# pyranha-labs/hypergrep

Measured on AMD Instinct MI355X. Metric: GiB/s scanned (256 patterns, 32 GiB synthetic log per GPU, text resident in HBM), higher is better.
Workload: dtype u8

## Files before the change

### hypergrep_amd/build.py

```python
from __future__ import annotations

import os
import shutil
import subprocess
import sys

PKG = os.path.dirname(os.path.abspath(__file__))
REPO = os.path.dirname(PKG)
CSRC = os.path.join(PKG, "csrc")
LIB_DIR = os.path.join(PKG, "lib")
LIB = os.path.join(LIB_DIR, "libhyperscanner.so")
LIBHS_NAME = "libhs.so.5"
OBJ = os.path.join(REPO, "build", "obj")
EXTRA = os.environ.get("HG_BUILD_DEFINES", "").split()
if os.environ.get("HG_BUILD_OUT"):
    LIB = os.path.abspath(os.environ["HG_BUILD_OUT"])
    LIB_DIR = os.path.dirname(LIB)
    OBJ = LIB + ".obj"
    LIBHS_NAME = os.path.basename(LIB) + ".libhs.so.5"

HIP_SOURCES = ["hg_stream.hip", "hg_kernels.hip", "hg_always_on.hip", "hg_huge.hip", "hg_som.hip", "hg_comb.hip", "hg_flows.hip", "hg_batch.hip", "hg_engine.hip", "hg_capi.hip", "hg_shim.hip", "hg_hsface.hip"]
CXX_SOURCES = ["hg_compile.cpp"]
HEADERS = ["hg_mem.h", "hg_db.h", "hg_core.h", "hg_post.h", "hg_engine.h", "hg_compile.h", "hg_synth.h", "hg_confirm_dev.h", "hg_sink_dev.h", "hg_tables_dev.h", "hg_som.h", "hg_comb.h", "hg_flows.h", "hg_flow_rules.h", "hg_batch.h", "hg_batch_launch.h"]

# ... 44 lines not shown

def _merge_resources() -> None:
    import json

    table = {}
    for src in KERNEL_SOURCES:
        path = os.path.join(OBJ, src + ".resources.json")
        if os.path.exists(path):
            with open(path, encoding="utf-8") as f:
                table.update(json.load(f))
    with open(os.path.join(LIB_DIR, "kernel_resources.json"), "w", encoding="utf-8") as f:
        json.dump(table, f, indent=1, sort_keys=True)
    for kernel, res in table.items():
        if kernel.startswith("_Z16hg_stream_kernelILi") and "ELb0ELi0E" in kernel and res.get("ScratchSize [bytes/lane]", 0) > 16:
            raise RuntimeError(f"{kernel} uses {res['ScratchSize [bytes/lane]']} bytes of scratch per lane: the streaming hot path must stay in registers")
        if "hg_som_kernel" in kernel and res.get("ScratchSize [bytes/lane]", 0) > 0:
            raise RuntimeError(f"{kernel} uses {res['ScratchSize [bytes/lane]']} bytes of scratch per lane: the start-of-match walks keep their state in registers / LDS")
        if "hg_minlen_kernel" in kernel and res.get("ScratchSize [bytes/lane]", 0) > 0:
            raise RuntimeError(f"{kernel} uses {res['ScratchSize [bytes/lane]']} bytes of scratch per lane: the match-length walks keep their state in registers / LDS")
        if "hg_flow_som_kernel" in kernel and res.get("ScratchSize [bytes/lane]", 0) > 0:
            raise RuntimeError(f"{kernel} uses {res['ScratchSize [bytes/lane]']} bytes of scratch per lane: the stream-mode start-of-match lanes keep their starts in device memory")
        if "hg_block_batch_kernel" in kernel and (res.get("ScratchSize [bytes/lane]", 0) > 0 or res.get("VGPRs Spill", 0) > 0):
            raise RuntimeError(f"{kernel} uses {res['ScratchSize [bytes/lane]']} bytes of scratch per lane, {res['VGPRs Spill']} spilled VGPRs: the batched block scan keeps its automaton state in registers")
        if "hg_comb_kernel" in kernel and res.get("ScratchSize [bytes/lane]", 0) > 0:
            raise RuntimeError(f"{kernel} uses {res['ScratchSize [bytes/lane]']} bytes of scratch per lane: the combination pass keeps its evaluation stack in a register")


def build(verbose: bool = False, force: bool = False) -> str:
    from concurrent.futures import ThreadPoolExecutor

    os.makedirs(OBJ, exist_ok=True)
    os.makedirs(LIB_DIR, exist_ok=True)
    hipcc = _hipcc()
    common_deps = [os.path.join(CSRC, h) for h in HEADERS] + [os.path.join(REPO, "include", "hypergrep_amd.h")]
    objs, jobs = [], []
    for src in HIP_SOURCES + CXX_SOURCES:
        path = os.path.join(CSRC, src)
        if not os.path.exists(path):
            continue
        obj = os.path.join(OBJ, src + ".o")
        objs.append(obj)
        if force or _stale(obj, [path] + common_deps):
            if src.endswith(".hip"):
                cmd = [hipcc, "--offload-arch=gfx950", "-O3", "-std=c++17", "-fPIC", "-Wall", "-Wno-pass-failed"] + EXTRA + ["-c", path, "-o", obj]
            else:
                cmd = ["g++", "-O2", "-std=c++17", "-fPIC", "-Wall", "-Wextra", "-c", path, "-o", obj]
# ... 34 lines not shown
```

### hypergrep_amd/csrc/hg_engine.h

```cpp
#pragma once
#include <hip/hip_runtime.h>

#include <memory>
#include <string>

#include "../../include/hypergrep_amd.h"
#include "hg_compile.h"
#include "hg_core.h"
#include "hg_post.h"

#ifndef HG_STREAM_WG_WAVES
#define HG_STREAM_WG_WAVES 8
#endif
constexpr uint32_t HG_STREAM_WG_WAVES_DEFAULT = HG_STREAM_WG_WAVES;

constexpr uint32_t HG_CONFIRM_SPLIT = 4;
constexpr uint32_t HG_DEFER_SHARDS = 64;

struct HgDeferred {
  uint64_t pos;
  uint32_t pattern;
  uint32_t rank;
};
enum { HG_ST_MINLEN_KEPT = 16, HG_ST_FIN_TOTAL = 24, HG_ST_SELECTED = 28, HG_ST_FINAL = 32, HG_ST_WORDS = 36, HG_ST_ZERO_WORDS = 32,
       HG_ST_BLOCK_DONE = 40 };
enum { HG_CNT_CANDS = 0, HG_CNT_HITS = 1, HG_CNT_CAND_NEED = 2, HG_CNT_HIT_NEED = 3, HG_CNT_DEFER_NEED = 4,
       HG_CNT_HITS_WRAPPED = 5,
       HG_CNT_JOIN_TILES = 6,
       HG_CNT_WORDS = 8,
       HG_CNT_CURSOR0 = 64,
       HG_CNT_CURSORS = 64,
       HG_ST_ALLOC_WORDS = 128 };
constexpr uint32_t HG_STREAM_GRAB = 2 * HG_STREAM_WG_WAVES_DEFAULT;

constexpr uint32_t HG_FIN_MAX_BUCKETS = 1u << 22;
constexpr uint32_t HG_FIN_BUCKET_CAP = 4096;
constexpr uint32_t HG_FIN_MEDIUM_CAP = 512;

#ifndef HG_CONFIRM_THREADS
#define HG_CONFIRM_THREADS 128
#endif



struct HgStreamArgs {
  const uint8_t *text;
  uint64_t nbytes, tile_begin, tile_end;
  HgDbView db;
  const uint32_t *filter;
  const HgSlotInfo *ext;
  HgTileSum *sums;
  HgCand *cands;
  uint32_t *seg_count;
  uint32_t cand_seg_cap, filter_log2;
  uint32_t weights_a, weights_b;
  uint32_t filter_wide;
  uint32_t dense;
  uint32_t weights_c;
  uint32_t alone;
  uint32_t cursor_slot;
  uint32_t *counters;
};

struct HgConfirmArgs {
  const uint8_t *text;
  uint64_t nbytes, tile_begin, tile_end, bs1;
// ... 204 lines not shown
```

### hypergrep_amd/csrc/hg_engine.hip

```cpp
#include <algorithm>
#include <array>
#include <cstdio>
#include <cstdlib>
#include <cstring>
#include <memory>

#include "hg_engine.h"
#include "hg_mem.h"

#include <rocprim/rocprim.hpp>

bool hg_launch_stream(const HgStreamArgs &a, uint32_t grid, hipStream_t stream);
bool hg_launch_stream_join(const HgStreamArgs &a, uint32_t grid, hipStream_t stream);
int hg_stream_blocks_per_cu(uint32_t filter_log2, uint32_t filter_wide, uint32_t dense);
__global__ void hg_tile_reduce_kernel(const HgTileSum *sums, uint64_t tile_begin, uint64_t tile_end, uint64_t bs1, HgTileElem *agg);
__global__ void hg_tile_spine_kernel(const HgTileElem *agg, uint32_t nblocks, uint64_t bs1, HgTileBase *block_base, HgTileBase *state);
__global__ void hg_tile_apply_kernel(const HgTileSum *sums, uint64_t tile_begin, uint64_t tile_end, uint64_t bs1, const HgTileBase *block_base,
                                     HgTileBase *bases);
__global__ void hg_tile_inner_kernel(const uint8_t *text, HgTileSum *sums, uint64_t tile_begin, uint64_t tile_end, uint64_t bs1);
__global__ void hg_verify_kernel(HgConfirmArgs a);
__global__ void hg_confirm_fast_kernel(HgConfirmArgs a, uint32_t blocks_per_mode);
__global__ void hg_confirm_generic_kernel(HgConfirmArgs a);
__global__ void hg_always_on_kernel(HgConfirmArgs a, uint32_t first, uint32_t last);
__global__ void hg_always_on_fast_kernel(HgConfirmArgs a);
__global__ void hg_always_on_finish_kernel(HgConfirmArgs a);
__global__ void hg_block_mark_kernel(HgConfirmArgs a, uint32_t *pattern_flags);
__global__ void hg_block_scan_kernel(HgConfirmArgs a, const uint32_t *pattern_flags);
__global__ void hg_block_small_kernel(HgDbView db, const uint8_t *h_text, uint32_t length, HgHit *h_out, uint32_t seg_cap, uint32_t *h_counts, uint32_t *d_done,
                                      uint32_t *h_flag, uint32_t seq, uint32_t ppw);
__global__ void hg_reset_kernel(uint32_t *state, uint32_t state_words, HgTileBase *final_state, uint64_t carry_start, uint64_t first_piece, uint32_t *fill, uint32_t nb, uint32_t *defer_count,
                                uint32_t ndefer);
__global__ void hg_fin_sort_small_kernel(const HgHit *hits, uint32_t *idx, const uint32_t *fill, uint32_t b_lo, uint32_t b_hi, uint32_t cap, uint32_t id_bits,
                                         uint32_t to_bits, uint32_t *kept_count, uint32_t *big_list, uint32_t *big_count, uint32_t big_stride);
template <uint32_t LCAP, bool IN_LDS>
__global__ void hg_fin_sort_big_kernel(const HgHit *hits, uint32_t *idx, const uint32_t *fill, const uint32_t *big_list, const uint32_t *big_count, uint32_t cap,
                                       uint32_t id_bits, uint32_t to_bits, uint32_t *kept_count, uint32_t *overflow, uint64_t *scratch_key, uint32_t *scratch_idx);
template <uint32_t THREADS>
__global__ void hg_fin_scan_kernel(uint32_t *kept_count, uint32_t b_lo, uint32_t b_hi, uint32_t *total, const uint32_t *fill, uint32_t cap, uint32_t *part, uint32_t epoch);
__global__ void hg_confirm_literal_kernel(HgConfirmArgs a);
__global__ void hg_verify_lean_kernel(HgConfirmArgs a);
__global__ void hg_fin_gather_kernel(const HgHit *hits, const HgHitAux *aux, const uint32_t *idx, const uint32_t *kept_base, const uint32_t *total, uint32_t b_lo,
                                     uint32_t b_hi, uint32_t cap, HgHit *oh, HgHitAux *oa);
__global__ void hg_key_kernel(const HgHit *hits, const HgHitAux *aux, const HgPattern *patterns, uint32_t n, uint64_t *key, uint32_t *idx);
__global__ void hg_line_key_kernel(const HgHit *hits, const uint32_t *perm, uint32_t n, uint64_t *key);
__global__ void hg_offset_kernel(uint32_t *idx, uint32_t n, uint32_t add);
__global__ void hg_key_packed_kernel(const HgHit *hits, const HgHitAux *aux, const HgPattern *patterns, uint32_t n, uint32_t id_bits, uint32_t to_bits,
                                     uint64_t *key, uint32_t *idx);
__global__ void hg_keep_kernel(const HgHit *hits, const HgHitAux *aux, const uint32_t *perm, const HgPattern *patterns, uint32_t n, uint8_t *keep);
__global__ void hg_scatter_kernel(const HgHit *hits, const HgHitAux *aux, const uint32_t *perm, const uint8_t *keep, const uint32_t *pos, uint32_t n,
                                  HgHit *oh, HgHitAux *oa, uint32_t *count);

size_t hg_huge_lds_bytes(uint32_t nw_max, uint32_t stage_cap);
bool hg_launch_confirm_huge(const HgConfirmArgs &a, uint32_t grid, uint32_t nw_max, uint32_t stage_cap, void *claim, uint32_t claim_mask, hipStream_t stream);
bool hg_launch_always_on_huge(const HgConfirmArgs &a, uint32_t grid, uint32_t nw_max, uint32_t stage_cap, uint32_t first, uint32_t last, hipStream_t stream);
bool hg_launch_block_huge(const HgConfirmArgs &a, uint32_t grid, uint32_t nw_max, uint32_t stage_cap, const uint32_t *pattern_flags, hipStream_t stream);

namespace {
constexpr int TS_BLOCK_TILES = 1024;
constexpr int STREAM_WG_WAVES = HG_STREAM_WG_WAVES;

template <typename T>
hipError_t upload(void **dst, const std::vector<T> &src, const char *name) {
  size_t bytes = std::max<size_t>(src.size() * sizeof(T), 16);
// ... 198 lines not shown
  (void)rocprim::exclusive_scan(nullptr, t2, d_keep_, d_perm_a_, 0u, n, rocprim::plus<uint32_t>(), hipStream_t(nullptr));
  size_t t3 = 0;
  (void)rocprim::merge(nullptr, t3, d_key_a_, d_key_a_, d_key_b_, d_perm_a_, d_perm_a_, d_perm_b_, n, n, rocprim::less<uint64_t>(), hipStream_t(nullptr));
  size_t need = std::max(std::max(t1, t2), t3) + 256;
  if (need > temp_bytes_) {
    hgmem::dev_free(d_temp_, "d_temp_");
    d_temp_ = nullptr;
    HG_TRY(hgmem::dev_alloc(&d_temp_, need, "d_temp_"), "workspace alloc (sort)");
    temp_bytes_ = need;
  }
  return HG_OK;
}

int HgScanner::ensure(uint64_t nbytes) {
  uint64_t ntiles = std::max<uint64_t>((nbytes + HG_TILE_BYTES - 1) / HG_TILE_BYTES, 1);
  auto re = [&](auto *&ptr, size_t count, const char *name) { return fail(realloc_dev(ptr, count, name), "workspace alloc"); };
  if (ntiles > cap_tiles_) {
    uint64_t nblocks = (ntiles + TS_BLOCK_TILES - 1) / TS_BLOCK_TILES;
    if (re(d_sums_, ntiles, "d_sums_") || re(d_bases_, ntiles + 1, "d_bases_") || re(d_agg_, nblocks, "d_agg_") || re(d_block_base_, nblocks, "d_block_base_")) return HG_ERR_HIP;
    cap_tiles_ = ntiles;
  }
  if (!d_seg_count_) {
    max_segs_ = static_cast<uint32_t>(num_cus_) * 16;
    if (re(d_seg_count_, max_segs_, "d_seg_count_") || re(d_seg_count2_, max_segs_, "d_seg_count2_") || re(d_defer_count_, HG_CONFIRM_MODES * HG_DEFER_SHARDS, "d_defer_count_")) return HG_ERR_HIP;
  }
  uint64_t want = std::max<uint64_t>(nbytes / 1024, 1u << 16);
  if (cand_cap_ < want && alloc_cands(want)) return HG_ERR_HIP;
  if (hit_cap_ < want && alloc_hits(want)) return HG_ERR_HIP;
  return HG_OK;
}

enum { HG_SPLIT = 1000, HG_GROWN = 1001 };

struct HgScanner::PassPlan {
  const uint8_t *text;
  uint64_t nbytes, bs1, ntiles;
  PassRange range;
  bool block_mode, has_anchored;
  hipStream_t stream, side;
  uint32_t id_bits, to_bits, fin_shift = 10, fin_nb = 1, fin_cap;
  bool bucketed;
  uint32_t nchunks = 1;
  bool piped, split;
  uint64_t chunk_tiles;
  std::array<uint64_t, kMaxChunks + 1> cut;
  uint32_t wgs_alone, wgs_shared, joiner_wgs, wgs = 1;
  uint32_t cand_seg_cap[2];
// ... 221 lines not shown
  if (p.block_mode) {
    HG_TRY(hipMemsetAsync(d_pflags_, 0, db_->patterns.size() * 4, side), "memset pattern flags");
    if (p.has_anchored) hipLaunchKernelGGL(hg_block_mark_kernel, dim3(segs_c), dim3(256), 0, side, ca, d_pflags_);
    always_blocks = std::max<uint32_t>(static_cast<uint32_t>((db_->patterns.size() + 255) / 256), std::min<uint32_t>(db_->nhuge, 1024u));
    ca.hit_seg_cap = hit_cap_ / always_blocks;
    hipLaunchKernelGGL(hg_block_scan_kernel, dim3(static_cast<uint32_t>((db_->patterns.size() + 255) / 256)), dim3(256), 0, side, ca, d_pflags_);
    if (db_->nhuge && !hg_launch_block_huge(ca, std::min<uint32_t>(db_->nhuge, 1024u), db_->huge_max_nw, db_->huge_stage_words, d_pflags_, side)) return huge_lds_error();
    HG_TRY(hipGetLastError(), "block-mode launch");
    p.stage_blocks = std::max(confirm_blocks, always_blocks);
    return HG_OK;
  }
  const uint64_t span = t1 - t0;
  const uint32_t nblocks = static_cast<uint32_t>((span + TS_BLOCK_TILES - 1) / TS_BLOCK_TILES);
  if (p.bs1 < HG_TILE_BYTES) {
    uint32_t blocks = static_cast<uint32_t>(std::min<uint64_t>((span + 255) / 256, 4096));
    hipLaunchKernelGGL(hg_tile_inner_kernel, dim3(blocks), dim3(256), 0, side, p.text, d_sums_, t0, t1, p.bs1);
  }
  hipLaunchKernelGGL(hg_tile_reduce_kernel, dim3(nblocks), dim3(256), 0, side, d_sums_, t0, t1, p.bs1, d_agg_);
  hipLaunchKernelGGL(hg_tile_spine_kernel, dim3(1), dim3(256), 0, side, d_agg_, nblocks, p.bs1, d_block_base_, d_final_);
  hipLaunchKernelGGL(hg_tile_apply_kernel, dim3(nblocks), dim3(256), 0, side, d_sums_, t0, t1, p.bs1, d_block_base_, d_bases_);
  HG_TRY(hipGetLastError(), "tile scan launch");
  if (p.piped && c + 1 == p.nchunks) HG_TRY(hipEventRecord(ev_tile_done_, side), "event");
  if (p.has_anchored) {
    const uint32_t verify_blocks = segs_c * HG_CONFIRM_SPLIT;
    uint32_t fast_modes = 0;
    const uint32_t mode_mask = knobs_.confirm_mode_mask;
    for (uint32_t m = 0; m < 3; m++) fast_modes += (db_->n_confirm_mode[m] && ((mode_mask >> m) & 1u)) ? 1 : 0;
    uint32_t per_cu = c + 1 == p.nchunks ? 6 : 3;
    if (knobs_.confirm_blocks_per_cu) per_cu = static_cast<uint32_t>(knobs_.confirm_blocks_per_cu);
    const uint32_t mode_blocks = std::max<uint32_t>(HG_DEFER_SHARDS, static_cast<uint32_t>(num_cus_) * per_cu * (256 / HG_CONFIRM_THREADS));
    const uint32_t huge_blocks = db_->n_confirm_mode[4] ? std::max<uint32_t>(HG_DEFER_SHARDS, static_cast<uint32_t>(num_cus_) * static_cast<uint32_t>(std::max<size_t>(1, std::min<size_t>(8, (160u << 10) / std::max<size_t>(hg_huge_lds_bytes(db_->huge_max_nw, db_->huge_stage_words), 1))))) : 0u;
    confirm_blocks = std::max(std::max(mode_blocks * std::max(fast_modes, 1u), verify_blocks), huge_blocks);
    ca.hit_seg_cap = hit_cap_ / confirm_blocks;
    if (c > 0) HG_TRY(hipMemsetAsync(d_defer_count_, 0, HG_CONFIRM_MODES * HG_DEFER_SHARDS * 4, side), "memset deferred counts");
    if (ca.mode_present[1] || ca.mode_present[2]) hipLaunchKernelGGL(hg_verify_kernel, dim3(verify_blocks), dim3(256), 0, side, ca);
    else hipLaunchKernelGGL(hg_verify_lean_kernel, dim3(verify_blocks), dim3(256), 0, side, ca);
    const bool literal_only_set = ca.mode_present[0] && !ca.mode_present[1] && !ca.mode_present[2];
    if (literal_only_set) {
      hipLaunchKernelGGL(hg_confirm_literal_kernel, dim3(mode_blocks), dim3(256), 0, side, ca);
    } else if (fast_modes) {
      hipLaunchKernelGGL(hg_confirm_fast_kernel, dim3(mode_blocks * fast_modes), dim3(HG_CONFIRM_THREADS), 0, side, ca, mode_blocks);
    }
    if (db_->n_confirm_mode[3]) hipLaunchKernelGGL(hg_confirm_generic_kernel, dim3(mode_blocks), dim3(256), 0, side, ca);
    if (huge_blocks && ((mode_mask >> 4) & 1u)) {
      HG_TRY(hipMemsetAsync(d_huge_claim_, 0, huge_claim_slots_ * 8, side), "memset claim table");
      if (!hg_launch_confirm_huge(ca, huge_blocks, db_->huge_max_nw, db_->huge_stage_words, d_huge_claim_, static_cast<uint32_t>(huge_claim_slots_ - 1), side)) return huge_lds_error();
    }
    HG_TRY(hipGetLastError(), "confirm launch");
  }
  if (!db_->slow.empty()) {
    always_blocks = static_cast<uint32_t>(std::min<uint64_t>((span + 3) / 4, static_cast<uint64_t>(num_cus_) * 8));
    const uint32_t huge_always_blocks = db_->nslow_huge ? static_cast<uint32_t>(std::min<uint64_t>(span, static_cast<uint64_t>(num_cus_) * 16)) : 0u;
    ca.hit_seg_cap = hit_cap_ / std::max(always_blocks, huge_always_blocks);
    const uint32_t nfast = db_->nslow_fast, nhuge = db_->nslow_huge, nall = static_cast<uint32_t>(db_->slow.size()) - nhuge;
    if (nfast) {
      ca.deferred = d_deferred_;
      ca.always_count = seg_count;
      ca.always_list_cap = cand_cap_ / always_blocks;
      hipLaunchKernelGGL(hg_always_on_fast_kernel, dim3(always_blocks), dim3(256), 0, side, ca);
// ... 166 lines not shown
    HG_TRY(realloc_dev(d_minlen_aux_, cap, "d_minlen_aux_"), "alloc (match-length pass)");
    minlen_cap_ = cap;
  }
  HG_TRY(hg_minlen_launch(text, d_hits_raw_, d_aux_raw_, *n, static_cast<const HgPattern *>(d_patterns_), static_cast<const uint32_t *>(d_pool_), minlen_max_nw_,
                          d_min_lengths_, d_minlen_hits_, d_minlen_aux_, d_counters_ + HG_ST_MINLEN_KEPT, stream),
         "match-length launch");
  HG_TRY(hipMemcpyAsync(h_counters_ + HG_ST_MINLEN_KEPT, d_counters_ + HG_ST_MINLEN_KEPT, 4, hipMemcpyDeviceToHost, stream), "copy count");
  HG_TRY(hipStreamSynchronize(stream), "stream sync (match-length pass)");
  *n = h_counters_[HG_ST_MINLEN_KEPT];
  return HG_OK;
}

int HgScanner::run_once(const uint8_t *text, uint64_t nbytes, uint64_t bs1, uint64_t line_base, const PassRange &range, bool block_mode, hipStream_t stream,
                        HgScanOutput *out) {
  if (range.tile_hi > range.tile_lo && stream_wgs_per_cu_ == 0) stream_wgs_per_cu_ = hg_stream_blocks_per_cu(db_->filter_log2, db_->filter_wide, db_->dense);
  PassPlan p = plan_pass(text, nbytes, bs1, line_base, range, block_mode, stream);
  HG_TRY(hipEventRecord(ev_[0], stream), "event");
  if (p.ntiles && !fin_fallback_ && p.fin_nb > fin_alloc_)
    if (int rc = alloc_fin(p.fin_nb, stream)) return rc;
  p.bucketed = p.bucketed && d_fin_fill_;
  p.ca.bucket_cap = p.bucketed ? p.fin_cap : 0u;
  p.ca.bucket_fill = d_fin_fill_;
  hipLaunchKernelGGL(hg_reset_kernel, dim3(std::max<uint32_t>(1, std::min<uint32_t>((p.fin_nb + 255) / 256, 256))), dim3(256), 0, stream, d_counters_, static_cast<uint32_t>(HG_ST_ZERO_WORDS), d_final_,
                     range.cs0, range.piece0, d_fin_fill_, p.bucketed ? p.fin_nb : 0u, d_defer_count_, static_cast<uint32_t>(HG_CONFIRM_MODES * HG_DEFER_SHARDS));
  HG_TRY(hipGetLastError(), "reset launch");
  if (p.split) return HG_SPLIT;
  out->stream_launches = p.ntiles ? p.nchunks : 0;
  if (p.ntiles) {
    if (p.piped && !ev_side_done_[0])
      for (int i = 0; i < kMaxChunks; i++) {
        HG_TRY(hipEventCreate(&ev_k1_begin_[i]), "hipEventCreate");
        HG_TRY(hipEventCreate(&ev_k1_end_[i]), "hipEventCreate");
        HG_TRY(hipEventCreate(&ev_side_done_[i]), "hipEventCreate");
      }
    if (p.piped) {
      HG_TRY(hipEventRecord(ev_side_done_[kMaxChunks - 1], stream), "event");
      HG_TRY(hipStreamWaitEvent(p.side, ev_side_done_[kMaxChunks - 1], 0), "stream wait");
    }
    for (uint32_t c = 0; c < p.nchunks; c++) {
      if (p.piped && c >= 2) HG_TRY(hipStreamWaitEvent(stream, ev_side_done_[c - 2], 0), "stream wait");
      if (int rc = launch_stream(p, c, out)) return rc;
      if (int rc = launch_side(p, c)) return rc;
      if (p.bucketed && c + 1 == p.nchunks)
        if (int rc = finalize_last(p, c)) return rc;
      if (p.piped) HG_TRY(hipEventRecord(ev_side_done_[c], p.side), "event");
    }
    if (p.piped) HG_TRY(hipStreamWaitEvent(stream, ev_side_done_[p.nchunks - 1], 0), "stream wait");
// ... 183 lines not shown
```

### hypergrep_amd/csrc/hg_kernels.hip

```cpp
#include <hip/hip_runtime.h>
#include <cstdlib>

#include "hg_confirm_dev.h"
#include "hg_core.h"
#include "hg_engine.h"
#include "hg_post.h"
#include "hg_sink_dev.h"
#include "hg_tables_dev.h"

namespace {

__device__ __forceinline__ uint32_t wave_inclusive_scan(uint32_t v, uint32_t lane) {
#pragma unroll
  for (int o = 1; o < 64; o <<= 1) {
    uint32_t u = __shfl_up(v, o, 64);
    if (lane >= static_cast<uint32_t>(o)) v += u;
  }
  return v;
}

}

namespace {
constexpr int TS_THREADS = 256;
// ... 74 lines not shown
  HgTileElem v = thread_elems(sums, tile_end, first, bs1, each);
  block_scan(v, sh, bs1);
  HgTileElem excl = identity_elem();
  if (threadIdx.x > 0) excl = sh[threadIdx.x - 1];
  HgTileBase st = hg_tile_apply(block_base[blockIdx.x], excl, bs1);
  for (int k = 0; k < TS_PER_THREAD; k++) {
    uint64_t t = first + k;
    if (t < tile_end) bases[t] = st;
    st = hg_tile_apply(st, each[k], bs1);
  }
}

__global__ __launch_bounds__(256) void hg_tile_inner_kernel(const uint8_t *text, HgTileSum *sums, uint64_t tile_begin, uint64_t tile_end, uint64_t bs1) {
  for (uint64_t t = tile_begin + static_cast<uint64_t>(blockIdx.x) * blockDim.x + threadIdx.x; t < tile_end; t += static_cast<uint64_t>(gridDim.x) * blockDim.x) {
    HgTileSum s = sums[t];
    if (s.nl_count < 2) continue;
    uint64_t base = t << HG_TILE_SHIFT;
    sums[t].inner = static_cast<uint32_t>(hg_inner_pieces(text, base + s.first_nl + 1, base + s.last_nl + 1, bs1));
  }
}

typedef uint32_t hg_u32x4_unaligned __attribute__((ext_vector_type(4), aligned(1)));

constexpr uint32_t VERIFY_STAGE_CAP = 768;
struct VerifyStage {
  HgDeferred item[VERIFY_STAGE_CAP];
  uint8_t bin[VERIFY_STAGE_CAP];
  uint32_t n;
  uint32_t bin_count[2 * HG_DEFER_SHARDS], bin_base[2 * HG_DEFER_SHARDS];
};
__device__ __forceinline__ void verify_stage_flush(const HgConfirmArgs &a, VerifyStage &st) {
  __syncthreads();
  const uint32_t n = st.n < VERIFY_STAGE_CAP ? st.n : VERIFY_STAGE_CAP;
  if (threadIdx.x < 2 * HG_DEFER_SHARDS) st.bin_count[threadIdx.x] = 0;
  __syncthreads();
  constexpr uint32_t PER_THREAD = (VERIFY_STAGE_CAP + 255) / 256;
  uint32_t rank[PER_THREAD];
#pragma unroll
  for (uint32_t q = 0; q < PER_THREAD; q++) {
    const uint32_t i = threadIdx.x + q * 256u;
    rank[q] = i < n ? atomicAdd(&st.bin_count[st.bin[i]], 1u) : 0u;
  }
  __syncthreads();
  if (threadIdx.x < 2 * HG_DEFER_SHARDS && st.bin_count[threadIdx.x])
    st.bin_base[threadIdx.x] = atomicAdd(&a.defer_count[HG_DEFER_SHARDS + threadIdx.x], st.bin_count[threadIdx.x]);
  __syncthreads();
#pragma unroll
  for (uint32_t q = 0; q < PER_THREAD; q++) {
    const uint32_t i = threadIdx.x + q * 256u;
    if (i < n) {
      const uint32_t bin = st.bin[i], m = 1u + bin / HG_DEFER_SHARDS, list = bin % HG_DEFER_SHARDS;
      const uint32_t slot = st.bin_base[bin] + rank[q];
      if (slot < a.defer_shard_cap) a.deferred[(static_cast<uint64_t>(a.list_of_mode[m]) * HG_DEFER_SHARDS + list) * a.defer_shard_cap + slot] = st.item[i];
      else atomicMax(&a.counters[HG_CNT_DEFER_NEED], slot + 1);
    }
  }
  __syncthreads();
  if (threadIdx.x == 0) st.n = 0;
  __syncthreads();
}

__device__ __forceinline__ uint32_t wtab_lookup(const HgWinBucket *tab, uint32_t bucket_mask, uint32_t folded) {
  for (uint32_t b = hg_wtab_bucket(folded, bucket_mask);; b = (b + 1u) & bucket_mask) {
    const uint4 *e = reinterpret_cast<const uint4 *>(tab + b);
    uint4 v = e[0], p = e[1];
    asm volatile("" : "+v"(v.x), "+v"(v.y), "+v"(v.z), "+v"(v.w), "+v"(p.x), "+v"(p.y), "+v"(p.z), "+v"(p.w));
    if (v.x == folded) return p.x;
    if (v.y == folded) return p.y;
    if (v.z == folded) return p.z;
    if (v.w == folded) return p.w;
    if (p.w == HG_WTAB_EMPTY) return HG_WTAB_EMPTY;
  }
}
__device__ __forceinline__ bool literal_occurs(const HgFactor *f, uint32_t len, const uint8_t *text, uint64_t fs, uint64_t readable) {
  const uint8_t *tp = text + fs;
  const uint32_t cb = f->casebits;
  uint32_t diff = 0;
  if (fs + (len > 16 ? 32u : 16u) <= readable) {
    const uint4 l0 = *reinterpret_cast<const uint4 *>(f->lit);
    const hg_u32x4_unaligned x0 = *reinterpret_cast<const hg_u32x4_unaligned *>(tp);
    diff = ((x0[0] ^ l0.x) & hg_factor_mask_dword(cb, len, 0)) | ((x0[1] ^ l0.y) & hg_factor_mask_dword(cb, len, 1)) |
           ((x0[2] ^ l0.z) & hg_factor_mask_dword(cb, len, 2)) | ((x0[3] ^ l0.w) & hg_factor_mask_dword(cb, len, 3));
    if (len > 16) {
      const uint4 l1 = *reinterpret_cast<const uint4 *>(f->lit + 16);
      const hg_u32x4_unaligned x1 = *reinterpret_cast<const hg_u32x4_unaligned *>(tp + 16);
      diff |= ((x1[0] ^ l1.x) & hg_factor_mask_dword(cb, len, 4)) | ((x1[1] ^ l1.y) & hg_factor_mask_dword(cb, len, 5)) |
              ((x1[2] ^ l1.z) & hg_factor_mask_dword(cb, len, 6)) | ((x1[3] ^ l1.w) & hg_factor_mask_dword(cb, len, 7));
    }
  } else {
    for (uint32_t b = 0; b < len; b++) diff |= (tp[b] ^ f->lit[b]) & (((cb >> b) & 1u) ? 0xDFu : 0xFFu);
  }
  return diff == 0;
}

template <bool STAGED>
__device__ __forceinline__ void verify_body(const HgConfirmArgs &a, VerifyStage *stage) {
  VerifyStage &s_stage = *stage;
  if (STAGED) {
    if (threadIdx.x == 0) s_stage.n = 0;
    __syncthreads();
  }
  const uint32_t lane = threadIdx.x & 63u, wave = threadIdx.x >> 6;
#ifdef HG_PROFILE_CONFIRM
  const uint64_t pf_t0 = wall_clock64();
  uint32_t pf_rounds = 0, pf_pairs = 0;
#endif
  const uint32_t seg = blockIdx.x / HG_CONFIRM_SPLIT, sub = blockIdx.x % HG_CONFIRM_SPLIT;
  const bool joined = seg >= a.join_seg0;
  const uint32_t seg_cap = joined ? a.join_seg_cap : a.cand_seg_cap;
  const HgCand *cseg = joined ? a.cands + static_cast<uint64_t>(a.join_seg0) * a.cand_seg_cap + static_cast<uint64_t>(seg - a.join_seg0) * a.join_seg_cap
                              : a.cands + static_cast<uint64_t>(seg) * a.cand_seg_cap;
  uint32_t n = a.seg_count[seg];
  if (n > seg_cap) n = seg_cap;
  const uint32_t shard = blockIdx.x % HG_DEFER_SHARDS;
  const uint32_t fold = a.db.fold_mask;
  const uint64_t readable = (a.nbytes + 15) & ~15ull;
  for (uint32_t base0 = sub * 256u; base0 < n; base0 += HG_CONFIRM_SPLIT * 256u) {
    if (STAGED) {
      __syncthreads();
      const uint32_t staged = s_stage.n;
      __syncthreads();
      if (staged >= VERIFY_STAGE_CAP / 2) verify_stage_flush(a, s_stage);
    }
    const uint32_t base = base0 + wave * 64u;
    const uint32_t i = base + lane;
    HgCand c{0, 0, 0};
    uint32_t j0 = 0, cnt = 0, folded = 0, direct_fo = 0, disc_h = 0, disc_d = 0;
    bool direct = false, shared = false;
    if (i < n) {
      c = cseg[i];
      folded = (c.word | fold) & a.db.window_mask;
      disc_h = hg_hash_window(folded);
      disc_d = a.db.disc[disc_h];
      if (a.db.wtab_first) {
        direct_fo = wtab_lookup(a.db.wtab, a.db.wtab_mask, folded);
        shared = direct_fo == HG_WTAB_SHARED;
        direct = !shared && direct_fo != HG_WTAB_EMPTY;
      } else {
        shared = true;
      }
      if (direct) cnt = 1;
    }
    if (shared) {
      const uint32_t h = disc_h;
      const uint32_t d = disc_d;
      const uint32_t sel = d >> 8;
      uint32_t key = 0;
      bool inside = true;
      if (sel) {
        const int64_t at = static_cast<int64_t>(c.pos) + static_cast<int8_t>(d & 0xFFu);
        const uint32_t lo = hg_ctz(sel), hi = 31u - hg_clz32(sel);
        inside = at + static_cast<int64_t>(lo) >= 0 && static_cast<uint64_t>(at + hi) < a.nbytes;
        if (inside) {
          uint32_t v = 0;
          if (at >= 0 && (at & 3) == 0) {
            v = *reinterpret_cast<const uint32_t *>(a.text + at);
          } else {
            for (uint32_t b = lo; b <= hi; b++) v |= static_cast<uint32_t>(a.text[at + static_cast<int64_t>(b)]) << (8u * b);
          }
          key = (v | fold) & hg_disc_bytes(sel);
        }
      }
      if (inside) {
        const uint32_t h2 = hg_disc_bucket(h, key);
        j0 = a.db.bucket_off2[h2];
        cnt = a.db.bucket_off2[h2 + 1] - j0;
      }
    }
    const uint32_t incl = wave_inclusive_scan(cnt, lane), start = incl - cnt;
    const uint32_t total = __shfl(incl, 63, 64);
#ifdef HG_PROFILE_CONFIRM
    pf_rounds++;
    pf_pairs += total;
#endif
    const uint32_t pos_lo = static_cast<uint32_t>(c.pos), pos_hi = static_cast<uint32_t>(c.pos >> 32);
    for (uint32_t t0 = 0; t0 < total; t0 += 64) {
      const uint32_t t = t0 + lane;
      uint32_t owner = 0;
#pragma unroll
      for (uint32_t step = 32; step; step >>= 1) {
        const uint32_t probe = owner + step;
        const uint32_t sp = __shfl(start, probe & 63u, 64);
        if (probe < 64u && sp <= t) owner = probe;
      }
      const uint32_t o_start = __shfl(start, owner, 64), o_j0 = __shfl(j0, owner, 64), o_folded = __shfl(folded, owner, 64);
      const uint32_t o_direct = __shfl(direct ? 1u : 0u, owner, 64), o_fo = __shfl(direct_fo, owner, 64);
      const uint32_t o_rank = __shfl(c.rank, owner, 64);
      const uint64_t pos = (static_cast<uint64_t>(static_cast<uint32_t>(__shfl(pos_hi, owner, 64))) << 32) | static_cast<uint32_t>(__shfl(pos_lo, owner, 64));
      bool ok = false;
      uint32_t mode = 0, tag = 0, mode_rank = 0;
      if (t < total) {
        HgWindow win{o_folded, o_fo};
        if (!o_direct) win = a.db.windows2[o_j0 + (t - o_start)];
        if (win.value == o_folded) {
          const uint32_t off = win.factor_off & 0xffu;
          const HgFactor *f = &a.db.factors[win.factor_off >> 8];
          const uint4 hdr = *reinterpret_cast<const uint4 *>(f);
          const uint32_t len = hdr.y;
          if (pos >= off && pos - off + len <= a.nbytes) {
            const uint64_t fs = pos - off;
            const uint32_t diff = literal_occurs(f, len, a.text, fs, readable) ? 0u : 1u;
            if (diff == 0) {
              ok = true;
              mode = hdr.z;
              mode_rank = hdr.w;
              tag = hdr.x | (off << 24);
            }
          }
        }
      }
      if (!__builtin_amdgcn_ballot_w64(ok)) continue;
#pragma unroll
      for (uint32_t m = 0; m < HG_CONFIRM_MODES; m++) {
        const uint64_t mm = __builtin_amdgcn_ballot_w64(ok && mode == m);
        if (!mm) continue;
        if (STAGED && (m == 1 || m == 2)) {
          uint32_t at0 = 0;
          if (lane == 0) at0 = atomicAdd(&s_stage.n, static_cast<uint32_t>(__popcll(mm)));
          at0 = __builtin_amdgcn_readfirstlane(at0);
          if (ok && mode == m) {
            const uint32_t at = at0 + __builtin_amdgcn_mbcnt_hi(static_cast<uint32_t>(mm >> 32), __builtin_amdgcn_mbcnt_lo(static_cast<uint32_t>(mm), 0u));
            const uint32_t list = (mode_rank * a.list_spread[m] + blockIdx.x % a.list_spread[m]) % HG_DEFER_SHARDS;
            if (at < VERIFY_STAGE_CAP) {
              s_stage.item[at] = HgDeferred{pos, tag, o_rank};
              s_stage.bin[at] = static_cast<uint8_t>((m - 1u) * HG_DEFER_SHARDS + list);
            } else {
              const uint32_t slot = atomicAdd(&a.defer_count[m * HG_DEFER_SHARDS + list], 1u);
              if (slot < a.defer_shard_cap) a.deferred[(static_cast<uint64_t>(a.list_of_mode[m]) * HG_DEFER_SHARDS + list) * a.defer_shard_cap + slot] = HgDeferred{pos, tag, o_rank};
              else atomicMax(&a.counters[HG_CNT_DEFER_NEED], slot + 1);
            }
          }
          continue;
        }
        uint32_t slot0 = 0;
        if (lane == 0) slot0 = atomicAdd(&a.defer_count[m * HG_DEFER_SHARDS + shard], static_cast<uint32_t>(__popcll(mm)));
        slot0 = __builtin_amdgcn_readfirstlane(slot0);
        if (ok && mode == m) {
          const uint32_t slot = slot0 + __builtin_amdgcn_mbcnt_hi(static_cast<uint32_t>(mm >> 32), __builtin_amdgcn_mbcnt_lo(static_cast<uint32_t>(mm), 0u));
          if (slot < a.defer_shard_cap) a.deferred[(static_cast<uint64_t>(a.list_of_mode[m]) * HG_DEFER_SHARDS + shard) * a.defer_shard_cap + slot] = HgDeferred{pos, tag, o_rank};
          else atomicMax(&a.counters[HG_CNT_DEFER_NEED], slot + 1);
        }
      }
    }
  }
  if (STAGED) verify_stage_flush(a, s_stage);
#ifdef HG_PROFILE_CONFIRM
  if (lane == 0) a.tmp_hits[(6u << 20) + 65536u + blockIdx.x * 4u + wave] = HgHit{pf_t0, static_cast<uint32_t>(wall_clock64() - pf_t0), pf_rounds | (pf_pairs << 8)};
#endif
}
#ifndef HG_VERIFY_WAVES
#define HG_VERIFY_WAVES 4
#endif
#ifndef HG_LITERAL_WAVES
#define HG_LITERAL_WAVES 3
#endif
__global__ __launch_bounds__(256) __attribute__((amdgpu_waves_per_eu(HG_VERIFY_WAVES, HG_VERIFY_WAVES))) void hg_verify_kernel(HgConfirmArgs a) {
  __shared__ VerifyStage s_stage;
  verify_body<true>(a, &s_stage);
}
__global__ __launch_bounds__(256) __attribute__((amdgpu_waves_per_eu(HG_VERIFY_WAVES, HG_VERIFY_WAVES))) void hg_verify_lean_kernel(HgConfirmArgs a) { verify_body<false>(a, nullptr); }

template <int MODE>
__device__ __forceinline__ void confirm_body(const HgConfirmArgs &a, uint32_t vblock, uint32_t vgrid) {
  __shared__ uint32_t s_n, s_base;
  if (threadIdx.x == 0) s_n = 0;
  __syncthreads();
  const uint64_t seg0 = static_cast<uint64_t>(blockIdx.x) * a.hit_seg_cap;
  const HitSink sink{a.tmp_hits + seg0, a.tmp_aux + seg0, a.hit_seg_cap, &s_n};
  const uint32_t shard = vblock % HG_DEFER_SHARDS, peer = vblock / HG_DEFER_SHARDS, peers = (vgrid + HG_DEFER_SHARDS - 1 - shard) / HG_DEFER_SHARDS;
  const HgDeferred *dlist = a.deferred + (static_cast<uint64_t>(a.list_of_mode[MODE]) * HG_DEFER_SHARDS + shard) * a.defer_shard_cap;
  uint32_t n = a.defer_count[MODE * HG_DEFER_SHARDS + shard];
  if (n > a.defer_shard_cap) n = a.defer_shard_cap;
  for (uint32_t i = peer * blockDim.x + threadIdx.x; i < n; i += peers * blockDim.x) {
    const HgDeferred d = dlist[i];
    const uint32_t pattern = d.pattern & (HG_MAX_PATTERNS - 1u);
    const HgPattern &p = a.db.patterns[pattern];
    const uint32_t id = p.id;
    const bool single = MODE != 3 || p.single != 0;
    auto emit = [&](uint64_t line_no, uint32_t to, uint64_t start, uint32_t len) { sink.push(a, line_no, id, to, start, len, pattern, single); };
    if (MODE == 0) hgdev::confirm_literal(a.text, a.nbytes, a.sums, a.bases, a.bs1, d.pos, d.rank, d.pos - (d.pattern >> 24), p.max_len, emit);
    else hg_confirm(a.db, a.text, a.nbytes, a.sums, a.bases, a.bs1, d.pos, pattern, d.rank, emit);
  }
  flush_hits(a, &s_n, &s_base);
// ... 505 lines not shown
```

Before: 5029.

## Balance verify pass with global candidate prefix and per-wave work stealing

The verify kernel no longer binds each block to one candidate segment. Every block builds an LDS prefix sum of segment fills, and each wave claims 64-candidate chunks from a global atomic cursor, then locates the owning segment by ballot and binary search. Staging of deferred items moves from a block-wide LDS buffer guarded by __syncthreads to per-wave buffers with wave barriers. Separate 'alone' kernel variants with different grid sizes and waves-per-EU are added for launches not overlapped with streaming. The aim is to remove load imbalance across skewed segments and block-level barriers, at the cost of per-block prefix construction, an extra cursor word, and atomic contention on that cursor.

```diff
diff --git a/hypergrep_amd/build.py b/hypergrep_amd/build.py
--- a/hypergrep_amd/build.py
+++ b/hypergrep_amd/build.py
@@ -90,6 +90,8 @@
             raise RuntimeError(f"{kernel} uses {res['ScratchSize [bytes/lane]']} bytes of scratch per lane: the stream-mode start-of-match lanes keep their starts in device memory")
         if "hg_block_batch_kernel" in kernel and (res.get("ScratchSize [bytes/lane]", 0) > 0 or res.get("VGPRs Spill", 0) > 0):
             raise RuntimeError(f"{kernel} uses {res['ScratchSize [bytes/lane]']} bytes of scratch per lane, {res['VGPRs Spill']} spilled VGPRs: the batched block scan keeps its automaton state in registers")
+        if "hg_verify_" in kernel and (res.get("ScratchSize [bytes/lane]", 0) > 0 or res.get("VGPRs Spill", 0) > 0):
+            raise RuntimeError(f"{kernel} uses {res['ScratchSize [bytes/lane]']} bytes of scratch per lane, {res['VGPRs Spill']} spilled VGPRs: neither instantiation of the verify pass (beside a stream launch, alone) may spill")
         if "hg_comb_kernel" in kernel and res.get("ScratchSize [bytes/lane]", 0) > 0:
             raise RuntimeError(f"{kernel} uses {res['ScratchSize [bytes/lane]']} bytes of scratch per lane: the combination pass keeps its evaluation stack in a register")
 
diff --git a/hypergrep_amd/csrc/hg_engine.h b/hypergrep_amd/csrc/hg_engine.h
--- a/hypergrep_amd/csrc/hg_engine.h
+++ b/hypergrep_amd/csrc/hg_engine.h
@@ -16,6 +16,7 @@
 
 constexpr uint32_t HG_CONFIRM_SPLIT = 4;
 constexpr uint32_t HG_DEFER_SHARDS = 64;
+constexpr uint32_t HG_VERIFY_ALONE_BLOCKS = 6, HG_VERIFY_LEAN_ALONE_BLOCKS = 8;
 
 struct HgDeferred {
   uint64_t pos;
@@ -42,6 +43,8 @@
 #endif
 
 
+
+constexpr uint32_t HG_DEFER_CURSOR = HG_CONFIRM_MODES * HG_DEFER_SHARDS, HG_DEFER_WORDS = HG_DEFER_CURSOR + 1;
 
 struct HgStreamArgs {
   const uint8_t *text;
diff --git a/hypergrep_amd/csrc/hg_engine.hip b/hypergrep_amd/csrc/hg_engine.hip
--- a/hypergrep_amd/csrc/hg_engine.hip
+++ b/hypergrep_amd/csrc/hg_engine.hip
@@ -18,7 +18,8 @@
 __global__ void hg_tile_apply_kernel(const HgTileSum *sums, uint64_t tile_begin, uint64_t tile_end, uint64_t bs1, const HgTileBase *block_base,
                                      HgTileBase *bases);
 __global__ void hg_tile_inner_kernel(const uint8_t *text, HgTileSum *sums, uint64_t tile_begin, uint64_t tile_end, uint64_t bs1);
-__global__ void hg_verify_kernel(HgConfirmArgs a);
+__global__ void hg_verify_kernel(HgConfirmArgs a, uint32_t nsegs);
+__global__ void hg_verify_alone_kernel(HgConfirmArgs a, uint32_t nsegs);
 __global__ void hg_confirm_fast_kernel(HgConfirmArgs a, uint32_t blocks_per_mode);
 __global__ void hg_confirm_generic_kernel(HgConfirmArgs a);
 __global__ void hg_always_on_kernel(HgConfirmArgs a, uint32_t first, uint32_t last);
@@ -38,7 +39,8 @@
 template <uint32_t THREADS>
 __global__ void hg_fin_scan_kernel(uint32_t *kept_count, uint32_t b_lo, uint32_t b_hi, uint32_t *total, const uint32_t *fill, uint32_t cap, uint32_t *part, uint32_t epoch);
 __global__ void hg_confirm_literal_kernel(HgConfirmArgs a);
-__global__ void hg_verify_lean_kernel(HgConfirmArgs a);
+__global__ void hg_verify_lean_kernel(HgConfirmArgs a, uint32_t nsegs);
+__global__ void hg_verify_lean_alone_kernel(HgConfirmArgs a, uint32_t nsegs);
 __global__ void hg_fin_gather_kernel(const HgHit *hits, const HgHitAux *aux, const uint32_t *idx, const uint32_t *kept_base, const uint32_t *total, uint32_t b_lo,
                                      uint32_t b_hi, uint32_t cap, HgHit *oh, HgHitAux *oa);
 __global__ void hg_key_kernel(const HgHit *hits, const HgHitAux *aux, const HgPattern *patterns, uint32_t n, uint64_t *key, uint32_t *idx);
@@ -283,7 +285,7 @@
   }
   if (!d_seg_count_) {
     max_segs_ = static_cast<uint32_t>(num_cus_) * 16;
-    if (re(d_seg_count_, max_segs_, "d_seg_count_") || re(d_seg_count2_, max_segs_, "d_seg_count2_") || re(d_defer_count_, HG_CONFIRM_MODES * HG_DEFER_SHARDS, "d_defer_count_")) return HG_ERR_HIP;
+    if (re(d_seg_count_, max_segs_, "d_seg_count_") || re(d_seg_count2_, max_segs_, "d_seg_count2_") || re(d_defer_count_, HG_DEFER_WORDS, "d_defer_count_")) return HG_ERR_HIP;
   }
   uint64_t want = std::max<uint64_t>(nbytes / 1024, 1u << 16);
   if (cand_cap_ < want && alloc_cands(want)) return HG_ERR_HIP;
@@ -551,7 +553,10 @@
   HG_TRY(hipGetLastError(), "tile scan launch");
   if (p.piped && c + 1 == p.nchunks) HG_TRY(hipEventRecord(ev_tile_done_, side), "event");
   if (p.has_anchored) {
-    const uint32_t verify_blocks = segs_c * HG_CONFIRM_SPLIT;
+    const bool alone = !p.piped || c + 1 == p.nchunks;
+    const bool staged = ca.mode_present[1] || ca.mode_present[2];
+    const uint32_t verify_blocks = static_cast<uint32_t>(num_cus_) * (!alone ? HG_CONFIRM_SPLIT : staged ? HG_VERIFY_ALONE_BLOCKS : HG_VERIFY_LEAN_ALONE_BLOCKS);
+    const uint32_t prefix_bytes = (segs_c + 1) * 4;
     uint32_t fast_modes = 0;
     const uint32_t mode_mask = knobs_.confirm_mode_mask;
     for (uint32_t m = 0; m < 3; m++) fast_modes += (db_->n_confirm_mode[m] && ((mode_mask >> m) & 1u)) ? 1 : 0;
@@ -561,9 +566,9 @@
     const uint32_t huge_blocks = db_->n_confirm_mode[4] ? std::max<uint32_t>(HG_DEFER_SHARDS, static_cast<uint32_t>(num_cus_) * static_cast<uint32_t>(std::max<size_t>(1, std::min<size_t>(8, (160u << 10) / std::max<size_t>(hg_huge_lds_bytes(db_->huge_max_nw, db_->huge_stage_words), 1))))) : 0u;
     confirm_blocks = std::max(std::max(mode_blocks * std::max(fast_modes, 1u), verify_blocks), huge_blocks);
     ca.hit_seg_cap = hit_cap_ / confirm_blocks;
-    if (c > 0) HG_TRY(hipMemsetAsync(d_defer_count_, 0, HG_CONFIRM_MODES * HG_DEFER_SHARDS * 4, side), "memset deferred counts");
-    if (ca.mode_present[1] || ca.mode_present[2]) hipLaunchKernelGGL(hg_verify_kernel, dim3(verify_blocks), dim3(256), 0, side, ca);
-    else hipLaunchKernelGGL(hg_verify_lean_kernel, dim3(verify_blocks), dim3(256), 0, side, ca);
+    if (c > 0) HG_TRY(hipMemsetAsync(d_defer_count_, 0, HG_DEFER_WORDS * 4, side), "memset deferred counts");
+    if (staged) hipLaunchKernelGGL(alone ? hg_verify_alone_kernel : hg_verify_kernel, dim3(verify_blocks), dim3(256), prefix_bytes, side, ca, segs_c);
+    else hipLaunchKernelGGL(alone ? hg_verify_lean_alone_kernel : hg_verify_lean_kernel, dim3(verify_blocks), dim3(256), prefix_bytes, side, ca, segs_c);
     const bool literal_only_set = ca.mode_present[0] && !ca.mode_present[1] && !ca.mode_present[2];
     if (literal_only_set) {
       hipLaunchKernelGGL(hg_confirm_literal_kernel, dim3(mode_blocks), dim3(256), 0, side, ca);
@@ -776,7 +781,7 @@
   p.ca.bucket_cap = p.bucketed ? p.fin_cap : 0u;
   p.ca.bucket_fill = d_fin_fill_;
   hipLaunchKernelGGL(hg_reset_kernel, dim3(std::max<uint32_t>(1, std::min<uint32_t>((p.fin_nb + 255) / 256, 256))), dim3(256), 0, stream, d_counters_, static_cast<uint32_t>(HG_ST_ZERO_WORDS), d_final_,
-                     range.cs0, range.piece0, d_fin_fill_, p.bucketed ? p.fin_nb : 0u, d_defer_count_, static_cast<uint32_t>(HG_CONFIRM_MODES * HG_DEFER_SHARDS));
+                     range.cs0, range.piece0, d_fin_fill_, p.bucketed ? p.fin_nb : 0u, d_defer_count_, HG_DEFER_WORDS);
   HG_TRY(hipGetLastError(), "reset launch");
   if (p.split) return HG_SPLIT;
   out->stream_launches = p.ntiles ? p.nchunks : 0;
diff --git a/hypergrep_amd/csrc/hg_kernels.hip b/hypergrep_amd/csrc/hg_kernels.hip
--- a/hypergrep_amd/csrc/hg_kernels.hip
+++ b/hypergrep_amd/csrc/hg_kernels.hip
@@ -120,42 +120,48 @@
 
 typedef uint32_t hg_u32x4_unaligned __attribute__((ext_vector_type(4), aligned(1)));
 
-constexpr uint32_t VERIFY_STAGE_CAP = 768;
+constexpr uint32_t VERIFY_STAGE_CAP = 512;
+constexpr uint32_t VERIFY_WAVE_CAP = VERIFY_STAGE_CAP / 4;
+static_assert(VERIFY_WAVE_CAP == 128, "verify_stage_flush: two staged occurrences and two bins per lane");
 struct VerifyStage {
-  HgDeferred item[VERIFY_STAGE_CAP];
-  uint8_t bin[VERIFY_STAGE_CAP];
-  uint32_t n;
-  uint32_t bin_count[2 * HG_DEFER_SHARDS], bin_base[2 * HG_DEFER_SHARDS];
+  HgDeferred item[VERIFY_WAVE_CAP];
+  uint32_t bin_slot[2 * HG_DEFER_SHARDS];
+  uint8_t bin[VERIFY_WAVE_CAP];
 };
-__device__ __forceinline__ void verify_stage_flush(const HgConfirmArgs &a, VerifyStage &st) {
-  __syncthreads();
-  const uint32_t n = st.n < VERIFY_STAGE_CAP ? st.n : VERIFY_STAGE_CAP;
-  if (threadIdx.x < 2 * HG_DEFER_SHARDS) st.bin_count[threadIdx.x] = 0;
-  __syncthreads();
-  constexpr uint32_t PER_THREAD = (VERIFY_STAGE_CAP + 255) / 256;
-  uint32_t rank[PER_THREAD];
+__device__ __forceinline__ void wave_lds_sync() {
+  __builtin_amdgcn_fence(__ATOMIC_SEQ_CST, "wavefront");
+  __builtin_amdgcn_wave_barrier();
+}
+__device__ __forceinline__ void verify_stage_flush(const HgConfirmArgs &a, VerifyStage &st, uint32_t n, uint32_t lane) {
+  if (n > VERIFY_WAVE_CAP) n = VERIFY_WAVE_CAP;
+  st.bin_slot[lane] = 0;
+  st.bin_slot[lane + 64u] = 0;
+  wave_lds_sync();
+  uint32_t rank[2], bin[2];
 #pragma unroll
-  for (uint32_t q = 0; q < PER_THREAD; q++) {
-    const uint32_t i = threadIdx.x + q * 256u;
-    rank[q] = i < n ? atomicAdd(&st.bin_count[st.bin[i]], 1u) : 0u;
-  }
-  __syncthreads();
-  if (threadIdx.x < 2 * HG_DEFER_SHARDS && st.bin_count[threadIdx.x])
-    st.bin_base[threadIdx.x] = atomicAdd(&a.defer_count[HG_DEFER_SHARDS + threadIdx.x], st.bin_count[threadIdx.x]);
-  __syncthreads();
+  for (uint32_t q = 0; q < 2; q++) {
+    const uint32_t i = lane + q * 64u;
+    bin[q] = i < n ? st.bin[i] : 0u;
+    rank[q] = i < n ? atomicAdd(&st.bin_slot[bin[q]], 1u) : 0u;
+  }
+  wave_lds_sync();
 #pragma unroll
-  for (uint32_t q = 0; q < PER_THREAD; q++) {
-    const uint32_t i = threadIdx.x + q * 256u;
+  for (uint32_t q = 0; q < 2; q++) {
+    const uint32_t b = lane + q * 64u, cnt = st.bin_slot[b];
+    if (cnt) st.bin_slot[b] = atomicAdd(&a.defer_count[HG_DEFER_SHARDS + b], cnt);
+  }
+  wave_lds_sync();
+#pragma unroll
+  for (uint32_t q = 0; q < 2; q++) {
+    const uint32_t i = lane + q * 64u;
     if (i < n) {
-      const uint32_t bin = st.bin[i], m = 1u + bin / HG_DEFER_SHARDS, list = bin % HG_DEFER_SHARDS;
-      const uint32_t slot = st.bin_base[bin] + rank[q];
+      const uint32_t m = 1u + bin[q] / HG_DEFER_SHARDS, list = bin[q] % HG_DEFER_SHARDS;
+      const uint32_t slot = st.bin_slot[bin[q]] + rank[q];
       if (slot < a.defer_shard_cap) a.deferred[(static_cast<uint64_t>(a.list_of_mode[m]) * HG_DEFER_SHARDS + list) * a.defer_shard_cap + slot] = st.item[i];
       else atomicMax(&a.counters[HG_CNT_DEFER_NEED], slot + 1);
     }
   }
-  __syncthreads();
-  if (threadIdx.x == 0) st.n = 0;
-  __syncthreads();
+  wave_lds_sync();
 }
 
 __device__ __forceinline__ uint32_t wtab_lookup(const HgWinBucket *tab, uint32_t bucket_mask, uint32_t folded) {
@@ -191,42 +197,100 @@
   return diff == 0;
 }
 
+extern __shared__ uint32_t s_seg_prefix[];
+__device__ __forceinline__ uint32_t verify_seg_fill(const HgConfirmArgs &a, uint32_t seg) {
+  const uint32_t n = a.seg_count[seg], cap = seg >= a.join_seg0 ? a.join_seg_cap : a.cand_seg_cap;
+  return n < cap ? n : cap;
+}
+__device__ __forceinline__ void verify_build_prefix(const HgConfirmArgs &a, uint32_t nsegs, uint32_t *prefix) {
+  __shared__ uint32_t s_wave_total[4];
+  const uint32_t lane = threadIdx.x & 63u, wave = threadIdx.x >> 6;
+  const uint32_t per = (nsegs + 255u) / 256u, first = threadIdx.x * per;
+  uint32_t sum = 0;
+  for (uint32_t k = 0; k < per; k++)
+    if (first + k < nsegs) sum += verify_seg_fill(a, first + k);
+  const uint32_t incl = wave_inclusive_scan(sum, lane);
+  if (lane == 63) s_wave_total[wave] = incl;
+  __syncthreads();
+  uint32_t at = incl - sum;
+  for (uint32_t w = 0; w < wave; w++) at += s_wave_total[w];
+  for (uint32_t k = 0; k < per; k++)
+    if (first + k < nsegs) {
+      prefix[first + k] = at;
+      at += verify_seg_fill(a, first + k);
+    }
+  if (threadIdx.x == 255) prefix[nsegs] = at;
+  __syncthreads();
+}
+
 template <bool STAGED>
-__device__ __forceinline__ void verify_body(const HgConfirmArgs &a, VerifyStage *stage) {
-  VerifyStage &s_stage = *stage;
-  if (STAGED) {
-    if (threadIdx.x == 0) s_stage.n = 0;
-    __syncthreads();
-  }
+__device__ __forceinline__ void verify_body(const HgConfirmArgs &a, uint32_t nsegs, VerifyStage *stage) {
   const uint32_t lane = threadIdx.x & 63u, wave = threadIdx.x >> 6;
+  uint32_t *prefix = s_seg_prefix;
+  verify_build_prefix(a, nsegs, prefix);
+  VerifyStage &s_stage = stage[STAGED ? wave : 0];
+  uint32_t staged = 0;
 #ifdef HG_PROFILE_CONFIRM
   const uint64_t pf_t0 = wall_clock64();
   uint32_t pf_rounds = 0, pf_pairs = 0;
 #endif
-  const uint32_t seg = blockIdx.x / HG_CONFIRM_SPLIT, sub = blockIdx.x % HG_CONFIRM_SPLIT;
-  const bool joined = seg >= a.join_seg0;
-  const uint32_t seg_cap = joined ? a.join_seg_cap : a.cand_seg_cap;
-  const HgCand *cseg = joined ? a.cands + static_cast<uint64_t>(a.join_seg0) * a.cand_seg_cap + static_cast<uint64_t>(seg - a.join_seg0) * a.join_seg_cap
-                              : a.cands + static_cast<uint64_t>(seg) * a.cand_seg_cap;
-  uint32_t n = a.seg_count[seg];
-  if (n > seg_cap) n = seg_cap;
+  const uint32_t ncand = prefix[nsegs];
+  const uint32_t coarse = (nsegs + 64u) / 64u;
   const uint32_t shard = blockIdx.x % HG_DEFER_SHARDS;
   const uint32_t fold = a.db.fold_mask;
   const uint64_t readable = (a.nbytes + 15) & ~15ull;
-  for (uint32_t base0 = sub * 256u; base0 < n; base0 += HG_CONFIRM_SPLIT * 256u) {
-    if (STAGED) {
-      __syncthreads();
-      const uint32_t staged = s_stage.n;
-      __syncthreads();
-      if (staged >= VERIFY_STAGE_CAP / 2) verify_stage_flush(a, s_stage);
-    }
-    const uint32_t base = base0 + wave * 64u;
-    const uint32_t i = base + lane;
+  uint32_t *cursor = a.defer_count + HG_DEFER_CURSOR;
+  uint32_t drawn = lane == 0 ? atomicAdd(cursor, 1u) : 0u;
+  for (;;) {
+    const uint64_t g0_wide = static_cast<uint64_t>(__builtin_amdgcn_readfirstlane(drawn)) * 64u;
+    if (g0_wide >= ncand) break;
+    drawn = lane == 0 ? atomicAdd(cursor, 1u) : 0u;
+    const uint32_t g0 = static_cast<uint32_t>(g0_wide);
+    if (STAGED && staged >= VERIFY_WAVE_CAP / 2) {
+      verify_stage_flush(a, s_stage, staged, lane);
+      staged = 0;
+    }
+    uint32_t s0;
+    {
+      const uint32_t probe = lane * coarse;
+      const uint32_t group = static_cast<uint32_t>(__popcll(__builtin_amdgcn_ballot_w64(probe <= nsegs && prefix[probe <= nsegs ? probe : nsegs] <= g0))) - 1u;
+      const uint32_t first = group * coarse;
+      s0 = first;
+      for (uint32_t off = 0; off < coarse; off += 64u) {
+        const uint32_t p2 = first + off + lane;
+        const uint32_t hold = static_cast<uint32_t>(__popcll(__builtin_amdgcn_ballot_w64(off + lane < coarse && p2 <= nsegs && prefix[p2 <= nsegs ? p2 : nsegs] <= g0)));
+        if (hold) s0 = first + off + hold - 1u;
+        if (hold < 64u) break;
+      }
+    }
+    const uint32_t g = g0 + lane;
+    const bool valid = g < ncand;
+    const uint32_t seg_start_l = prefix[s0 + lane < nsegs ? s0 + lane : nsegs];
+    uint32_t k = 0;
+#pragma unroll
+    for (uint32_t step = 32; step; step >>= 1) {
+      const uint32_t probe = k + step;
+      const uint32_t sp = __shfl(seg_start_l, probe & 63u, 64);
+      if (probe < 64u && sp <= g) k = probe;
+    }
+    uint32_t seg = s0 + k, seg_start = __shfl(seg_start_l, k, 64);
+    if (valid && k == 63u) {
+      uint32_t lo = seg, hi = nsegs;
+      while (hi - lo > 1u) {
+        const uint32_t mid = (lo + hi) >> 1;
+        if (prefix[mid] <= g) lo = mid;
+        else hi = mid;
+      }
+      seg = lo;
+      seg_start = prefix[lo];
+    }
     HgCand c{0, 0, 0};
     uint32_t j0 = 0, cnt = 0, folded = 0, direct_fo = 0, disc_h = 0, disc_d = 0;
     bool direct = false, shared = false;
-    if (i < n) {
-      c = cseg[i];
+    if (valid) {
+      const bool joined = seg >= a.join_seg0;
+      const uint64_t at = joined ? static_cast<uint64_t>(a.join_seg0) * a.cand_seg_cap + static_cast<uint64_t>(seg - a.join_seg0) * a.join_seg_cap : static_cast<uint64_t>(seg) * a.cand_seg_cap;
+      c = a.cands[at + (g - seg_start)];
       folded = (c.word | fold) & a.db.window_mask;
       disc_h = hg_hash_window(folded);
       disc_d = a.db.disc[disc_h];
@@ -269,7 +333,7 @@
     const uint32_t total = __shfl(incl, 63, 64);
 #ifdef HG_PROFILE_CONFIRM
     pf_rounds++;
-    pf_pairs += total;
+    pf_pairs += static_cast<uint32_t>(__popcll(__builtin_amdgcn_ballot_w64(valid)));
 #endif
     const uint32_t pos_lo = static_cast<uint32_t>(c.pos), pos_hi = static_cast<uint32_t>(c.pos >> 32);
     for (uint32_t t0 = 0; t0 < total; t0 += 64) {
@@ -313,13 +377,12 @@
         const uint64_t mm = __builtin_amdgcn_ballot_w64(ok && mode == m);
         if (!mm) continue;
         if (STAGED && (m == 1 || m == 2)) {
-          uint32_t at0 = 0;
-          if (lane == 0) at0 = atomicAdd(&s_stage.n, static_cast<uint32_t>(__popcll(mm)));
-          at0 = __builtin_amdgcn_readfirstlane(at0);
+          const uint32_t at0 = staged;
+          staged += static_cast<uint32_t>(__popcll(mm));
           if (ok && mode == m) {
             const uint32_t at = at0 + __builtin_amdgcn_mbcnt_hi(static_cast<uint32_t>(mm >> 32), __builtin_amdgcn_mbcnt_lo(static_cast<uint32_t>(mm), 0u));
             const uint32_t list = (mode_rank * a.list_spread[m] + blockIdx.x % a.list_spread[m]) % HG_DEFER_SHARDS;
-            if (at < VERIFY_STAGE_CAP) {
+            if (at < VERIFY_WAVE_CAP) {
               s_stage.item[at] = HgDeferred{pos, tag, o_rank};
               s_stage.bin[at] = static_cast<uint8_t>((m - 1u) * HG_DEFER_SHARDS + list);
             } else {
@@ -341,7 +404,7 @@
       }
     }
   }
-  if (STAGED) verify_stage_flush(a, s_stage);
+  if (STAGED && staged) verify_stage_flush(a, s_stage, staged, lane);
 #ifdef HG_PROFILE_CONFIRM
   if (lane == 0) a.tmp_hits[(6u << 20) + 65536u + blockIdx.x * 4u + wave] = HgHit{pf_t0, static_cast<uint32_t>(wall_clock64() - pf_t0), pf_rounds | (pf_pairs << 8)};
 #endif
@@ -352,11 +415,16 @@
 #ifndef HG_LITERAL_WAVES
 #define HG_LITERAL_WAVES 3
 #endif
-__global__ __launch_bounds__(256) __attribute__((amdgpu_waves_per_eu(HG_VERIFY_WAVES, HG_VERIFY_WAVES))) void hg_verify_kernel(HgConfirmArgs a) {
-  __shared__ VerifyStage s_stage;
-  verify_body<true>(a, &s_stage);
-}
-__global__ __launch_bounds__(256) __attribute__((amdgpu_waves_per_eu(HG_VERIFY_WAVES, HG_VERIFY_WAVES))) void hg_verify_lean_kernel(HgConfirmArgs a) { verify_body<false>(a, nullptr); }
+__global__ __launch_bounds__(256) __attribute__((amdgpu_waves_per_eu(HG_VERIFY_WAVES, HG_VERIFY_WAVES))) void hg_verify_kernel(HgConfirmArgs a, uint32_t nsegs) {
+  __shared__ VerifyStage s_stage[4];
+  verify_body<true>(a, nsegs, s_stage);
+}
+__global__ __launch_bounds__(256) __attribute__((amdgpu_waves_per_eu(HG_VERIFY_WAVES, HG_VERIFY_WAVES))) void hg_verify_lean_kernel(HgConfirmArgs a, uint32_t nsegs) { verify_body<false>(a, nsegs, nullptr); }
+__global__ __launch_bounds__(256) __attribute__((amdgpu_waves_per_eu(HG_VERIFY_ALONE_BLOCKS))) void hg_verify_alone_kernel(HgConfirmArgs a, uint32_t nsegs) {
+  __shared__ VerifyStage s_stage[4];
+  verify_body<true>(a, nsegs, s_stage);
+}
+__global__ __launch_bounds__(256) __attribute__((amdgpu_waves_per_eu(HG_VERIFY_LEAN_ALONE_BLOCKS))) void hg_verify_lean_alone_kernel(HgConfirmArgs a, uint32_t nsegs) { verify_body<false>(a, nsegs, nullptr); }
 
 template <int MODE>
 __device__ __forceinline__ void confirm_body(const HgConfirmArgs &a, uint32_t vblock, uint32_t vgrid) {
```

Result: slower. 4752 (-5.5%).
